# kchmck/p25rx

Measured on NVIDIA B200. Metric: Msamples/s IQ demod+decode (real-time P25 channels = baseband samples/s / 48000), higher is better.
Workload: dtype f32

## Files before the change

p25rx_b200/csrc/ddc_fm.cu:

```cuda
#include "p25cu_internal.cuh"
#include "p25_imma_tables.h"

__constant__ float c_taps_front[P25_TAPS_FRONT];
__constant__ float c_taps_decim[P25_TAPS_DECIM];
__constant__ float c_taps_chan[P25_TAPS_CHAN];
__constant__ float c_iq_lut[256];

static_assert(P25_TAPS_FRONT == 5 * P25_DECIM_FRONT, "front stage is a 10-phase x 5-tap polyphase matrix");
static_assert(P25_TAPS_DECIM == 5 * P25_DECIM_NATIVE, "decimator is a 5-phase x 5-tap polyphase matrix");

template <bool FRONT>
struct Cfg {
    static constexpr int MB = FRONT ? 64 : 256;
    static constexpr int NT = FRONT ? 320 : 256;
    static constexpr int DIN = FRONT ? 50 : 5;
    static constexpr int XN = MB * DIN;
    static constexpr int ACOLS = FRONT ? 5 * MB : 0;
    static constexpr int RING = FRONT ? 128 : 512;
    static constexpr int HT = FRONT ? 3264 : 1312;
};

template <bool FRONT>
struct Smem {
    using C = Cfg<FRONT>;
    float2 xs[C::XN];
    float2 pa[2][4][FRONT ? C::ACOLS : 1];
    float ya_re[FRONT ? C::ACOLS : 1], ya_im[FRONT ? C::ACOLS : 1];
    float2 pd[2][4][C::MB];
    float yd_re[C::RING], yd_im[C::RING];
    float c_re[C::RING], c_im[C::RING];
    float d[C::RING];
    float red[32];
    float lut[256];
};

template <int FMT>
struct Elem { using T = float2; };
template <>
struct Elem<P25CU_FMT_U8_IQ> { using T = uchar2; };

template <int FMT>
__device__ __forceinline__ float2 cvt(const float* lut, typename Elem<FMT>::T v) {
    if constexpr (FMT == P25CU_FMT_CF32_IQ) return v;
    else return make_float2(lut[v.x], lut[v.y]);
}

template <int FMT>
__device__ __forceinline__ typename Elem<FMT>::T load_logical_raw(const DdcParams& p, const void* tail, const void* chunk, long long l) {
    using T = typename Elem<FMT>::T;
    if (l < (long long)p.ht) return ((const T*)tail)[l];
    const long long i = l - p.ht;
    if (i >= (long long)p.n) return T{};
    return __ldcs((const T*)chunk + i);
}

template <bool FRONT, int FMT>
__device__ __forceinline__ void stage_block(Smem<FRONT>& sm, const DdcParams& p, const void* tail, const void* chunk,
                                            long long l0) {
    using C = Cfg<FRONT>;
    const long long ht = (long long)p.ht;
    const int tid = threadIdx.x;
    const long long t_end = l0 + C::XN < ht ? l0 + C::XN : ht;
    if (l0 < t_end) {
        if constexpr (FMT == P25CU_FMT_CF32_IQ) {
            for (long long l = (l0 & ~1LL) + 2 * tid; l < t_end; l += 2 * C::NT) {
                const float4 v = *(const float4*)((const float2*)tail + l);
                const long long i = l - l0;
                if (i >= 0) sm.xs[i] = make_float2(v.x, v.y);
                if (i + 1 < C::XN && l + 1 < t_end) sm.xs[i + 1] = make_float2(v.z, v.w);
            }
        } else {
            const long long zero_below = ht - (long long)p.a0;
            for (long long l = l0 + tid; l < t_end; l += C::NT) {
                const uchar2 b = ((const uchar2*)tail)[l];
                sm.xs[l - l0] = l < zero_below ? make_float2(0.f, 0.f) : make_float2(sm.lut[b.x], sm.lut[b.y]);
            }
        }
    }
    const long long c_beg = (l0 > ht ? l0 : ht) - ht, c_end = l0 + C::XN - ht;
    if (c_end <= c_beg) return;
    const long long base = ht - l0;
    const long long n = (long long)p.n;
    if (p.aligned16) {
        if (FMT == P25CU_FMT_CF32_IQ) {
            for (long long g = (c_beg & ~1LL) + 2 * tid; g < c_end; g += 2 * C::NT) {
                const float4 v = g < n ? __ldcs((const float4*)((const float2*)chunk + g)) : make_float4(0.f, 0.f, 0.f, 0.f);
                if (g >= c_beg) sm.xs[g + base] = make_float2(v.x, v.y);
                if (g + 1 < c_end) sm.xs[g + 1 + base] = make_float2(v.z, v.w);
            }
        } else {
            for (long long g = (c_beg & ~7LL) + 8 * tid; g < c_end; g += 8 * C::NT) {
                const uint4 v = g < n ? __ldcs((const uint4*)((const uchar2*)chunk + g)) : make_uint4(0x7F7F7F7Fu, 0x7F7F7F7Fu, 0x7F7F7F7Fu, 0x7F7F7F7Fu);
                const unsigned w[4] = {v.x, v.y, v.z, v.w};
#pragma unroll
                for (int e = 0; e < 8; e++) {
                    const long long jj = g + e;
                    if (jj >= c_beg && jj < c_end) {
                        const unsigned b = w[e >> 1] >> (16 * (e & 1));
                        sm.xs[jj + base] = jj < n ? make_float2(sm.lut[b & 0xFF], sm.lut[(b >> 8) & 0xFF]) : make_float2(0.f, 0.f);
                    }
                }
            }
        }
    } else {
        for (long long jj = c_beg + tid; jj < c_end; jj += C::NT) {
            float2 v = make_float2(0.f, 0.f);
            if (jj < n) v = cvt<FMT>(sm.lut, __ldcs((const typename Elem<FMT>::T*)chunk + jj));
            sm.xs[jj + base] = v;
        }
    }
}

template <int D>
__device__ __forceinline__ void column_partials(const float2 (&x)[D], const float* __restrict__ h, float2 (&P)[5]) {
#pragma unroll
    for (int q = 0; q < 5; q++) {
        float re = 0.f, im = 0.f;
#pragma unroll
        for (int pp = 0; pp < D; pp++) {
            const float t = h[D * q + pp];
            re = fmaf(t, x[D - 1 - pp].x, re);
            im = fmaf(t, x[D - 1 - pp].y, im);
        }
        P[q] = make_float2(re, im);
    }
}

template <bool FRONT, int FMT>
__global__ void __launch_bounds__(Cfg<FRONT>::NT) p25_ddc_fm_kernel(const DdcParams p) {
    using C = Cfg<FRONT>;
    extern __shared__ __align__(16) unsigned char smem_raw[];
    Smem<FRONT>& sm = *reinterpret_cast<Smem<FRONT>*>(smem_raw);
    const int tid = threadIdx.x;
    const unsigned s = blockIdx.x / p.n_seg, g = blockIdx.x % p.n_seg;

    {
        float* z = reinterpret_cast<float*>(&sm.pa[0][0][0]);
        const int nz = (int)((sizeof(Smem<FRONT>) - sizeof(sm.xs) - sizeof(sm.lut)) / sizeof(float));
        for (int i = tid; i < nz; i += C::NT) z[i] = 0.f;
        for (int i = tid; i < 256; i += C::NT) sm.lut[i] = c_iq_lut[i];
    }

    using ET = typename Elem<FMT>::T;
    const void* tail = (const ET*)p.tail_in + (size_t)s * p.ht;
    const void* chunk = (FMT == P25CU_FMT_CF32_IQ) ? (const void*)((const float2*)p.iq + (size_t)s * p.n)
                                                    : (const void*)((const uchar2*)p.iq + (size_t)s * p.n);
    float* out = p.bb + (size_t)s * p.row_stride + P25CU_BB_HIST;

    const long long M0 = (long long)p.m0;
    const long long mb = M0 + (long long)g * p.seg_out;
    long long me = mb + p.seg_out;
    if (me > M0 + (long long)p.n_out) me = M0 + p.n_out;
    const long long a0 = (long long)p.a0;
    float pw = 0.f;
    int pb = 0;
    __syncthreads();

    for (long long mi = mb - C::MB; mi < me; mi += C::MB, pb ^= 1) {
        stage_block<FRONT, FMT>(sm, p, tail, chunk, (long long)C::DIN * mi - a0 + (long long)p.ht);
        __syncthreads();

        if constexpr (FRONT) {
            float2 P[5];
            {
                float2 x[10];
                const float4* src = reinterpret_cast<const float4*>(&sm.xs[10 * tid]);
#pragma unroll
                for (int i = 0; i < 5; i++) {
                    const float4 v = src[i];
                    x[2 * i] = make_float2(v.x, v.y);
                    x[2 * i + 1] = make_float2(v.z, v.w);
                }
                column_partials<10>(x, c_taps_front, P);
            }
#pragma unroll
            for (int q = 1; q < 5; q++) sm.pa[pb][q - 1][tid] = P[q];
            __syncthreads();
            float re = P[0].x, im = P[0].y;
#pragma unroll
            for (int q = 1; q < 5; q++) {
                const int c = tid - q;
                const float2 v = c >= 0 ? sm.pa[pb][q - 1][c] : sm.pa[pb ^ 1][q - 1][C::ACOLS + c];
                re += v.x;
                im += v.y;
            }
            sm.ya_re[tid] = re;
            sm.ya_im[tid] = im;
            __syncthreads();
        }

        float2 Q[5];
        if (tid < C::MB) {
            float2 x[5];
            if constexpr (FRONT) {
#pragma unroll
                for (int i = 0; i < 5; i++) x[i] = make_float2(sm.ya_re[5 * tid + i], sm.ya_im[5 * tid + i]);
            } else {
#pragma unroll
                for (int i = 0; i < 5; i++) x[i] = sm.xs[5 * tid + i];
            }
            column_partials<5>(x, c_taps_decim, Q);
#pragma unroll
            for (int q = 1; q < 5; q++) sm.pd[pb][q - 1][tid] = Q[q];
        }
        __syncthreads();
        if (tid < C::MB) {
            float re = Q[0].x, im = Q[0].y;
#pragma unroll
            for (int q = 1; q < 5; q++) {
                const int c = tid - q;
                const float2 v = c >= 0 ? sm.pd[pb][q - 1][c] : sm.pd[pb ^ 1][q - 1][C::MB + c];
                re += v.x;
                im += v.y;
            }
            const unsigned r = (unsigned)(mi + tid) & (C::RING - 1);
            sm.yd_re[r] = re;
            sm.yd_im[r] = im;
        }
        __syncthreads();

        for (int w = tid; w < 2 * C::MB; w += C::NT) {
            const int o = w < C::MB ? w : w - C::MB;
            const float* src = w < C::MB ? sm.yd_re : sm.yd_im;
            const unsigned r = (unsigned)(mi + o);
            float acc = 0.f;
#pragma unroll
            for (int k = 0; k < P25_TAPS_CHAN; k++) acc = fmaf(c_taps_chan[k], src[(r - k) & (C::RING - 1)], acc);
            (w < C::MB ? sm.c_re : sm.c_im)[r & (C::RING - 1)] = acc;
        }
        __syncthreads();

        if (tid < C::MB) {
            const long long m = mi + tid;
            const unsigned r = (unsigned)m;
            const float cr = sm.c_re[r & (C::RING - 1)], ci = sm.c_im[r & (C::RING - 1)];
            const float pr = sm.c_re[(r - 1) & (C::RING - 1)], pi = sm.c_im[(r - 1) & (C::RING - 1)];
            const float re = cr * pr + ci * pi;
            const float im = ci * pr - cr * pi;
            sm.d[r & (C::RING - 1)] = atan2f(im, re) * P25_FM_GAIN;
            if (m >= mb && m < me) pw += cr * cr + ci * ci;
        }
        __syncthreads();

        if (tid < C::MB) {
            const long long m = mi + tid;
            if (m >= mb && m < me) {
                const unsigned r = (unsigned)m;
                float acc = 0.f;
#pragma unroll
                for (int i = P25_BOXCAR - 1; i >= 0; i--) acc += sm.d[(r - i) & (C::RING - 1)];
                out[m - M0] = acc / (float)P25_BOXCAR;
            }
        }
    }

    if (p.power_sum) {
#pragma unroll
        for (int o = 16; o > 0; o >>= 1) pw += __shfl_xor_sync(0xFFFFFFFFu, pw, o);
        __syncthreads();
        if ((tid & 31) == 0) sm.red[tid >> 5] = pw;
        __syncthreads();
        if (tid == 0) {
            float t = 0.f;
            for (int i = 0; i < C::NT / 32; i++) t += sm.red[i];
            atomicAdd(p.power_sum + s, t);
        }
    }

    if (g == p.n_seg - 1) {
        ET* tout = (ET*)p.tail_out + (size_t)s * p.ht;
        for (int i = tid; i < (int)p.ht; i += C::NT) tout[i] = load_logical_raw<FMT>(p, tail, chunk, (long long)p.n + i);
    }
}

namespace fast {

constexpr int MB = 64;
constexpr int NT = 320;
constexpr int XN = MB * 50;
constexpr int ACOLS = 5 * MB;
constexpr int HC = P25_TAPS_CHAN - 1;
constexpr int HB = P25_BOXCAR - 1;

template <int FMT>
struct F {
    static constexpr bool U8 = FMT == P25CU_FMT_U8_IQ;
    static constexpr int ES = U8 ? 2 : 8;
    static constexpr int AL = U8 ? 8 : 2;
    static constexpr int XLEN = U8 ? XN + AL : XN;
    static constexpr int XBYTES = (XLEN * ES + 127) / 128 * 128;
#ifndef DDC50_MAXREG
#define DDC50_MAXREG 56
#endif
#ifndef DDC50_U8_MAXREG
#define DDC50_U8_MAXREG 48
#endif
    static constexpr int MAXREG = U8 ? DDC50_U8_MAXREG : DDC50_MAXREG;
};

template <int FMT>
struct __align__(128) Smem {
    unsigned char xs[2][F<FMT>::XBYTES];
    float2 pa[4][ACOLS + 4];
    float2 ya[ACOLS];
    float2 pd[4][MB + 4];
    float2 yd[HC + MB];
    float2 c[1 + MB];
    float d[HB + MB];
    float red[16];
    unsigned long long full[2];
};

__device__ __forceinline__ unsigned smem_u32(const void* p) { return (unsigned)__cvta_generic_to_shared(p); }
__device__ __forceinline__ void mbar_init(unsigned long long* bar, unsigned count) {
    asm volatile("mbarrier.init.shared::cta.b64 [%0], %1;" ::"r"(smem_u32(bar)), "r"(count));
}
__device__ __forceinline__ void mbar_expect_tx(unsigned long long* bar, unsigned bytes) {
    asm volatile("mbarrier.arrive.expect_tx.shared::cta.b64 _, [%0], %1;" ::"r"(smem_u32(bar)), "r"(bytes) : "memory");
}
__device__ __forceinline__ void mbar_wait(unsigned long long* bar, unsigned parity) {
    unsigned ok;
    do {
        asm volatile(
            "{\n\t.reg .pred p;\n\tmbarrier.try_wait.parity.shared::cta.b64 p, [%1], %2;\n\tselp.u32 %0, 1, 0, p;\n\t}"
            : "=r"(ok)
            : "r"(smem_u32(bar)), "r"(parity)
            : "memory");
    } while (!ok);
}
__device__ __forceinline__ void tma_load_1d(void* dst, const void* src, unsigned bytes, unsigned long long* bar) {
    asm volatile("cp.async.bulk.shared::cluster.global.mbarrier::complete_tx::bytes [%0], [%1], %2, [%3];" ::"r"(smem_u32(dst)),
                 "l"(src), "r"(bytes), "r"(smem_u32(bar))
                 : "memory");
}
__device__ __forceinline__ float2 cfma(float h, float2 x, float2 acc) {
    unsigned long long r;
    const float2 hh = make_float2(h, h);
    asm("fma.rn.f32x2 %0, %1, %2, %3;"
        : "=l"(r)
        : "l"(*reinterpret_cast<const unsigned long long*>(&hh)), "l"(*reinterpret_cast<const unsigned long long*>(&x)),
          "l"(*reinterpret_cast<const unsigned long long*>(&acc)));
    return *reinterpret_cast<float2*>(&r);
}
__device__ __forceinline__ float2 add2(float2 a, float2 b) {
    unsigned long long r;
    asm("add.rn.f32x2 %0, %1, %2;"
        : "=l"(r)
        : "l"(*reinterpret_cast<const unsigned long long*>(&a)), "l"(*reinterpret_cast<const unsigned long long*>(&b)));
    return *reinterpret_cast<float2*>(&r);
}

template <int NS, bool ODD>
__device__ __forceinline__ void load_u8n(const unsigned* __restrict__ wp, float2 (&x)[NS]) {
    constexpr int NWORD = (NS + (ODD ? 1 : 0) + 1) / 2;
    unsigned w[NWORD];
#pragma unroll
    for (int i = 0; i < NWORD; i++) w[i] = wp[i];
    const float2 off = make_float2(-8388736.f, -8388736.f);
#pragma unroll
    for (int i = 0; i < NS; i++) {
        const int hw = i + (ODD ? 1 : 0);
        const unsigned word = w[hw >> 1];
        const unsigned fi = __byte_perm(word, 0x4B000000u, (hw & 1) ? 0x7442u : 0x7440u);
        const unsigned fq = __byte_perm(word, 0x4B000000u, (hw & 1) ? 0x7443u : 0x7441u);
        x[i] = add2(make_float2(__uint_as_float(fi), __uint_as_float(fq)), off);
    }
}

template <int D>
__device__ __forceinline__ void partials(const float2 (&x)[D], const float* __restrict__ h, float2 (&P)[5]) {
#pragma unroll
    for (int q = 0; q < 5; q++) {
        float2 a = make_float2(0.f, 0.f);
#pragma unroll
        for (int pp = 0; pp < D; pp++) a = cfma(h[D * q + pp], x[D - 1 - pp], a);
        P[q] = a;
    }
}

template <int FMT>
__device__ __forceinline__ void issue_block(Smem<FMT>& sm, int stage, const DdcParams& p, const unsigned char* tail,
                                            const unsigned char* chunk, long long l0) {
    constexpr int ES = F<FMT>::ES;
    const long long ht = p.ht, lend = ht + (long long)p.n;
    const long long la = l0 & ~(long long)(F<FMT>::AL - 1);
    long long l1 = la + F<FMT>::XLEN;
    if (l1 > lend) l1 = lend;
    const long long t1 = l1 < ht ? l1 : ht;
    const unsigned nt = la < t1 ? (unsigned)(t1 - la) : 0u;
    const long long cb = la > ht ? la : ht;
    const unsigned nc = cb < l1 ? (unsigned)(l1 - cb) : 0u;
    mbar_expect_tx(&sm.full[stage], (nt + nc) * ES);
    if (nt) tma_load_1d(&sm.xs[stage][0], tail + la * ES, nt * ES, &sm.full[stage]);
    if (nc) tma_load_1d(&sm.xs[stage][(cb - la) * ES], chunk + (cb - ht) * ES, nc * ES, &sm.full[stage]);
}

#ifndef DDC50_DYN_CH
#define DDC50_DYN_CH 16
#endif
#ifndef DDC50_STATIC_NUM
#define DDC50_STATIC_NUM 7
#define DDC50_STATIC_DEN 8
#endif
constexpr unsigned DYN_CH = DDC50_DYN_CH;

template <int FMT>
__global__ void __maxnreg__(F<FMT>::MAXREG) p25_ddc_fm_stream_kernel(const DdcParams p, const unsigned blocks_per_stream,
                                                                    const unsigned n_static, const unsigned n_tickets,
                                                                    const unsigned ticket_base, const float dc, const float pw_scale) {
    constexpr int ES = F<FMT>::ES;
    extern __shared__ __align__(128) unsigned char smem_raw[];
    Smem<FMT>& sm = *reinterpret_cast<Smem<FMT>*>(smem_raw);
    __shared__ unsigned s_ticket;
    const int tid = threadIdx.x;

    if (tid == 0) {
        mbar_init(&sm.full[0], 1);
        mbar_init(&sm.full[1], 1);
        asm volatile("fence.mbarrier_init.release.cluster;" ::: "memory");
    }
    const unsigned long long total = (unsigned long long)p.n_streams * blocks_per_stream;
    const unsigned long long dyn_begin = (unsigned long long)n_static * gridDim.x;
    unsigned long long b = (unsigned long long)n_static * blockIdx.x;
    unsigned long long b_end = b + n_static;
    const long long M0 = (long long)p.m0, a0 = (long long)p.a0;
    unsigned use = 0;
    __syncthreads();

  for (;;) {
    if (b >= b_end) {
        if (tid == 0) s_ticket = atomicAdd(p.work_counter, 1u) - ticket_base;
        __syncthreads();
        const unsigned c = s_ticket;
        __syncthreads();
        if (c >= n_tickets) break;
        b = dyn_begin + (unsigned long long)c * DYN_CH;
        b_end = b + DYN_CH < total ? b + DYN_CH : total;
    }
    while (b < b_end) {
        const unsigned s = (unsigned)(b / blocks_per_stream);
        const unsigned it0 = (unsigned)(b % blocks_per_stream);
        unsigned it1 = blocks_per_stream;
        if (b_end - b < (unsigned long long)(it1 - it0)) it1 = it0 + (unsigned)(b_end - b);
        b += it1 - it0;
        const unsigned char* tail = (const unsigned char*)p.tail_in + (size_t)s * p.ht * ES;
        const unsigned char* chunk = (const unsigned char*)p.iq + (size_t)s * p.n * ES;
        const long long mb = M0 + (long long)it0 * MB;
        long long me = M0 + (long long)it1 * MB;
        if (me > M0 + (long long)p.n_out) me = M0 + p.n_out;
        float* out = p.bb + (size_t)s * p.row_stride + P25CU_BB_HIST - M0;
        const long long lbase = -a0 + (long long)p.ht;

        for (int i = tid; i < 4 * 4; i += NT) {
            sm.pa[i >> 2][i & 3] = make_float2(0.f, 0.f);
            sm.pd[i >> 2][i & 3] = make_float2(0.f, 0.f);
        }
        for (int i = tid; i < HC; i += NT) sm.yd[i] = make_float2(0.f, 0.f);
        if (tid == 0) sm.c[0] = make_float2(0.f, 0.f);
        if (tid < HB) sm.d[tid] = 0.f;
        float pw = 0.f;
        const long long m_first = mb - MB;
        const int nblk = (int)((me - m_first + MB - 1) / MB);
        if (tid == 0) {
            issue_block<FMT>(sm, use & 1, p, tail, chunk, 50 * m_first + lbase);
            if (nblk > 1) issue_block<FMT>(sm, (use + 1) & 1, p, tail, chunk, 50 * (m_first + MB) + lbase);
        }
        __syncthreads();

        for (int blk = 0; blk < nblk; blk++, use++) {
            const long long mi = m_first + (long long)blk * MB;
            const int stage = use & 1;
            mbar_wait(&sm.full[stage], (use >> 1) & 1);

            float2 P[5];
            {
                float2 x[10];
                if constexpr (F<FMT>::U8) {
                    const int s0 = (int)((50 * mi + lbase) & (F<FMT>::AL - 1)) + 10 * tid;
                    const unsigned* wp = reinterpret_cast<const unsigned*>(sm.xs[stage]) + (s0 >> 1);
                    if (s0 & 1) load_u8n<10, true>(wp, x);
                    else load_u8n<10, false>(wp, x);
                } else {
                    const float4* src = reinterpret_cast<const float4*>(sm.xs[stage]) + 5 * tid;
#pragma unroll
                    for (int i = 0; i < 5; i++) {
                        const float4 v = src[i];
                        x[2 * i] = make_float2(v.x, v.y);
                        x[2 * i + 1] = make_float2(v.z, v.w);
                    }
                }
                partials<10>(x, c_taps_front, P);
            }
#pragma unroll
            for (int q = 1; q < 5; q++) sm.pa[q - 1][tid + 4] = P[q];
            __syncthreads();
            if (tid == 0 && blk + 2 < nblk) issue_block<FMT>(sm, stage, p, tail, chunk, 50 * (mi + 2 * MB) + lbase);
            {
                float2 a = P[0];
#pragma unroll
                for (int q = 1; q < 5; q++) {
                    const float2 v = sm.pa[q - 1][tid + 4 - q];
                    a.x += v.x;
                    a.y += v.y;
                }
                sm.ya[tid] = a;
            }
            __syncthreads();
            if (tid >= ACOLS - 4) {
#pragma unroll
                for (int q = 1; q < 5; q++) sm.pa[q - 1][tid - (ACOLS - 4)] = P[q];
            }
            float2 Q[5];
            if (tid < MB) {
                float2 x[5];
#pragma unroll
                for (int i = 0; i < 5; i++) x[i] = sm.ya[5 * tid + i];
                partials<5>(x, c_taps_decim, Q);
#pragma unroll
                for (int q = 1; q < 5; q++) sm.pd[q - 1][tid + 4] = Q[q];
            }
            __syncthreads();
            if (tid < MB) {
                float2 a = Q[0];
#pragma unroll
                for (int q = 1; q < 5; q++) {
                    const float2 v = sm.pd[q - 1][tid + 4 - q];
                    a.x += v.x;
                    a.y += v.y;
                }
                sm.yd[HC + tid] = a;
            }
            __syncthreads();
            if (tid >= MB - 4 && tid < MB) {
#pragma unroll
                for (int q = 1; q < 5; q++) sm.pd[q - 1][tid - (MB - 4)] = Q[q];
            }
            if (tid < MB) {
                float2 e = make_float2(dc, dc), o = make_float2(0.f, 0.f);
                const float2* src = &sm.yd[HC + tid];
#pragma unroll
                for (int k = 0; k + 1 < P25_TAPS_CHAN; k += 2) {
                    e = cfma(c_taps_chan[k], src[-k], e);
                    o = cfma(c_taps_chan[k + 1], src[-k - 1], o);
                }
                e = cfma(c_taps_chan[P25_TAPS_CHAN - 1], src[-(P25_TAPS_CHAN - 1)], e);
                sm.c[1 + tid] = make_float2(e.x + o.x, e.y + o.y);
            }
            __syncthreads();
            if (tid < MB) {
                const float2 cur = sm.c[1 + tid], prv = sm.c[tid];
                const float re = cur.x * prv.x + cur.y * prv.y;
                const float im = cur.y * prv.x - cur.x * prv.y;
                sm.d[HB + tid] = atan2f(im, re) * P25_FM_GAIN;
                const long long m = mi + tid;
                if (m >= mb && m < me) pw += cur.x * cur.x + cur.y * cur.y;
            } else if (tid >= 128 && tid < 128 + HC) {
                sm.yd[tid - 128] = sm.yd[MB + tid - 128];
            }
            __syncthreads();
            float bsum = 0.f;
            if (tid < MB) {
#pragma unroll
                for (int i = 0; i < P25_BOXCAR; i++) bsum += sm.d[tid + i];
                const long long m = mi + tid;
                if (m >= mb && m < me) out[m] = bsum / (float)P25_BOXCAR;
            } else if (tid == 128) {
                sm.c[0] = sm.c[MB];
            }
            __syncthreads();
            if (tid < HB) sm.d[tid] = sm.d[MB + tid];
        }

        if (p.power_sum) {
#pragma unroll
            for (int o = 16; o > 0; o >>= 1) pw += __shfl_xor_sync(0xFFFFFFFFu, pw, o);
            if ((tid & 31) == 0) sm.red[tid >> 5] = pw;
            __syncthreads();
            if (tid == 0) {
                float t = 0.f;
                for (int i = 0; i < NT / 32; i++) t += sm.red[i];
                atomicAdd(p.power_sum + s, t * pw_scale);
            }
        }
        if (it1 == blocks_per_stream) {
            using ET = typename Elem<FMT>::T;
            ET* tout = (ET*)p.tail_out + (size_t)s * p.ht;
            for (int i = tid; i < (int)p.ht; i += NT)
                tout[i] = load_logical_raw<FMT>(p, tail, chunk, (long long)p.n + i);
        }
        __syncthreads();
    }
  }
}

__device__ __forceinline__ float2 mul2(float2 a, float2 b) {
    unsigned long long r;
    asm("mul.rn.f32x2 %0, %1, %2;"
        : "=l"(r)
        : "l"(*reinterpret_cast<const unsigned long long*>(&a)), "l"(*reinterpret_cast<const unsigned long long*>(&b)));
    return *reinterpret_cast<float2*>(&r);
}
__device__ __forceinline__ float2 fma2s(float2 a, float2 b, float c) {
    unsigned long long r;
    const float2 cc = make_float2(c, c);
    asm("fma.rn.f32x2 %0, %1, %2, %3;"
        : "=l"(r)
        : "l"(*reinterpret_cast<const unsigned long long*>(&a)), "l"(*reinterpret_cast<const unsigned long long*>(&b)),
          "l"(*reinterpret_cast<const unsigned long long*>(&cc)));
    return *reinterpret_cast<float2*>(&r);
}
__device__ __forceinline__ float2 disc_atan2_pair(float2 y, float2 x) {
    const float ax0 = fabsf(x.x), ay0 = fabsf(y.x), ax1 = fabsf(x.y), ay1 = fabsf(y.y);
    const float mx0 = fmaxf(ax0, ay0), mn0 = fminf(ax0, ay0), mx1 = fmaxf(ax1, ay1), mn1 = fminf(ax1, ay1);
    float rc0, rc1;
    asm("rcp.approx.ftz.f32 %0, %1;" : "=f"(rc0) : "f"(fmaxf(mx0, 1e-30f)));
    asm("rcp.approx.ftz.f32 %0, %1;" : "=f"(rc1) : "f"(fmaxf(mx1, 1e-30f)));
    const float2 t = mul2(make_float2(mn0, mn1), make_float2(rc0, rc1)), u = mul2(t, t);
    float2 q = make_float2(-0.004295386839658022f, -0.004295386839658022f);
    q = fma2s(q, u, 0.022737378254532814f);
    q = fma2s(q, u, -0.057179518043994904f);
    q = fma2s(q, u, 0.09735459089279175f);
    q = fma2s(q, u, -0.13945257663726807f);
    q = fma2s(q, u, 0.1995391547679901f);
    q = fma2s(q, u, -0.3333050608634949f);
    q = fma2s(q, u, 0.9999995231628418f);
    const float2 r = mul2(q, t);
    float r0 = r.x, r1 = r.y;
    r0 = ay0 > ax0 ? 1.57079632679489662f - r0 : r0;
    r1 = ay1 > ax1 ? 1.57079632679489662f - r1 : r1;
    r0 = x.x < 0.f ? 3.14159265358979324f - r0 : r0;
    r1 = x.y < 0.f ? 3.14159265358979324f - r1 : r1;
    return make_float2(copysignf(r0, y.x), copysignf(r1, y.y));
}

}


namespace w5 {

using fast::cfma;
using fast::mbar_init;
using fast::mbar_expect_tx;
using fast::mbar_wait;
using fast::tma_load_1d;
using fast::add2;
using fast::disc_atan2_pair;

constexpr int R = 4;
constexpr int NOUT = 31 * R;
constexpr int XNEW = 5 * NOUT;
constexpr int XN = 32 * 5 * R;
constexpr int WARPS = 4;
constexpr int AL = 2, ES = 8;
constexpr int XLEN = (XN + 2 * AL - 2) / AL * AL;
constexpr int XBYTES = (XLEN * ES + 127) / 128 * 128;
constexpr int MINB = 4;
constexpr int HROWS = (P25_TAPS_CHAN - 1) / R;
constexpr int DROWS = 3;
static_assert((P25_TAPS_CHAN - 1) % R == 0 && DROWS * R >= P25_BOXCAR - 1, "history rows");

struct __align__(128) WarpSm {
    unsigned char xs[2][XBYTES];
    float4 ydA[HROWS + 32], ydB[HROWS + 32];
    float4 d4[DROWS + 32];
    unsigned long long full[2];
};

__device__ __forceinline__ void issue_slice(WarpSm& sm, int stage, int ht, int lend, const unsigned char* tail,
                                            const unsigned char* chunk, int l0) {
    const int la = l0 & ~(AL - 1);
    const int lb = min(la + XLEN, lend);
    if (la >= ht) {
        const unsigned bytes = (unsigned)(lb - la) * ES;
        mbar_expect_tx(&sm.full[stage], bytes);
        tma_load_1d(&sm.xs[stage][0], chunk + (size_t)(la - ht) * ES, bytes, &sm.full[stage]);
        return;
    }
    const int t1 = min(lb, ht);
    const unsigned nt = (unsigned)(t1 - la), nc = (unsigned)(lb - t1);
    mbar_expect_tx(&sm.full[stage], (nt + nc) * ES);
    tma_load_1d(&sm.xs[stage][0], tail + (size_t)la * ES, nt * ES, &sm.full[stage]);
    if (nc) tma_load_1d(&sm.xs[stage][nt * ES], chunk, nc * ES, &sm.full[stage]);
}

__global__ void __launch_bounds__(32 * WARPS, MINB) p25_ddc5_warp_kernel(const DdcParams p, const unsigned its_per_stream,
                                                                         const float dc, const float pw_scale) {
    extern __shared__ __align__(128) unsigned char smem_raw[];
    const int lane = threadIdx.x & 31, warp = threadIdx.x >> 5;
    WarpSm& sm = reinterpret_cast<WarpSm*>(smem_raw)[warp];
    if (lane == 0) {
        mbar_init(&sm.full[0], 1);
        mbar_init(&sm.full[1], 1);
        asm volatile("fence.mbarrier_init.release.cluster;" ::: "memory");
    }
    for (int i = lane; i < HROWS + 32; i += 32) sm.ydA[i] = sm.ydB[i] = make_float4(0.f, 0.f, 0.f, 0.f);
    for (int i = lane; i < DROWS + 32; i += 32) sm.d4[i] = make_float4(0.f, 0.f, 0.f, 0.f);
    __syncwarp();

    const unsigned gw = blockIdx.x * WARPS + warp, GW = gridDim.x * WARPS;
    const unsigned long long total = (unsigned long long)p.n_streams * its_per_stream;
    const unsigned long long b0 = total * gw / GW, b1 = total * (gw + 1ull) / GW;
    if (b0 >= b1) return;
    const int ips = (int)its_per_stream, ht = (int)p.ht, lend = (int)p.ht + (int)p.n, n_out = (int)p.n_out;
    const size_t row_bytes = (size_t)p.n * ES, tail_bytes = (size_t)p.ht * ES;
    const int l_base = (int)(5 * (long long)p.m0 - (long long)p.a0) - 20 + ht;
    const bool want_pw = p.power_sum != nullptr;
    unsigned s = (unsigned)(b0 / its_per_stream);
    int it_first = (int)(b0 % its_per_stream);
    unsigned left = (unsigned)(b1 - b0);
    const unsigned char* chunk = (const unsigned char*)p.iq + s * row_bytes;
    const unsigned char* tail = (const unsigned char*)p.tail_in + s * tail_bytes;
    if (lane == 0) {
        issue_slice(sm, 0, ht, lend, tail, chunk, l_base + XNEW * (it_first - 1));
        issue_slice(sm, 1, ht, lend, tail, chunk, l_base + XNEW * it_first);
    }
    float2 c_carry = make_float2(0.f, 0.f);
    unsigned use = 0;

    while (left) {
      const int n_st = min(ips - it_first, (int)left);
      const int npiece = n_st + 1;
      left -= (unsigned)n_st;
      float* const out_lane = p.bb + (size_t)s * p.row_stride + P25CU_BB_HIST + R * lane;
      float pw = 0.f;
      for (int j = 0; j < npiece; j++, use++) {
        const int it = it_first - 1 + j;
        const int stage = use & 1;
        const int skew = (l_base + XNEW * it) & (AL - 1);
        const int nv = j ? min(n_out - NOUT * it, NOUT) : 0;
        mbar_wait(&sm.full[stage], (use >> 1) & 1);

        float2 own[R];
        {
            float2 x[5 * R];
            const int s0 = skew + 5 * R * lane;
            const float4* xp = reinterpret_cast<const float4*>(reinterpret_cast<const float2*>(sm.xs[stage]) + (s0 & ~1));
            if (s0 & 1) {
#pragma unroll
                for (int i = 0; i <= 5 * R / 2; i++) {
                    const float4 v = xp[i];
                    if (i > 0) x[2 * i - 1] = make_float2(v.x, v.y);
                    if (i < 5 * R / 2) x[2 * i] = make_float2(v.z, v.w);
                }
            } else {
#pragma unroll
                for (int i = 0; i < 5 * R / 2; i++) {
                    const float4 v = xp[i];
                    x[2 * i] = make_float2(v.x, v.y);
                    x[2 * i + 1] = make_float2(v.z, v.w);
                }
            }
            float2 lft[R];
#pragma unroll
            for (int r = 0; r < R; r++) {
                own[r] = make_float2(0.f, 0.f);
                lft[r] = make_float2(0.f, 0.f);
#pragma unroll
                for (int k = P25_TAPS_DECIM - 1; k >= 0; k--) {
                    if ((P25_TAPS_DECIM_ZERO_MASK >> k) & 1) continue;
                    const int idx = 5 * r + (P25_TAPS_DECIM - 1) - k;
                    if (idx < 5 * R) own[r] = cfma(c_taps_decim[k], x[idx], own[r]);
                    else lft[r] = cfma(c_taps_decim[k], x[idx - 5 * R], lft[r]);
                }
            }
#pragma unroll
            for (int r = 0; r < R; r++) {
                if (5 * r + (P25_TAPS_DECIM - 1) >= 5 * R) {
                    own[r].x += __shfl_down_sync(0xFFFFFFFFu, lft[r].x, 1);
                    own[r].y += __shfl_down_sync(0xFFFFFFFFu, lft[r].y, 1);
                }
            }
        }
        sm.ydA[HROWS + lane] = make_float4(own[0].x, own[0].y, own[1].x, own[1].y);
        sm.ydB[HROWS + lane] = make_float4(own[2].x, own[2].y, own[3].x, own[3].y);
        __syncwarp();
        if (lane == 0) {
            if (j + 2 < npiece) issue_slice(sm, stage, ht, lend, tail, chunk, l_base + XNEW * (it + 2));
            else if (left) issue_slice(sm, stage, ht, lend, tail + tail_bytes, chunk + row_bytes, l_base + XNEW * (j + 1 - npiece));
        }

        float2 acc[R];
#pragma unroll
        for (int r = 0; r < R; r++) acc[r] = make_float2(dc, dc);
#pragma unroll
        for (int t = 0; t <= HROWS; t++) {
            const float4 va = sm.ydA[lane + t], vb = sm.ydB[lane + t];
            const float2 xs4[4] = {make_float2(va.x, va.y), make_float2(va.z, va.w), make_float2(vb.x, vb.y), make_float2(vb.z, vb.w)};
#pragma unroll
            for (int q = 0; q < 4; q++) {
#pragma unroll
                for (int r = 0; r < R; r++) {
                    const int k = (P25_TAPS_CHAN - 1) + r - (4 * t + q);
                    if (k >= 0 && k < P25_TAPS_CHAN) acc[r] = cfma(c_taps_chan[k], xs4[q], acc[r]);
                }
            }
        }
        float2 prev;
        prev.x = __shfl_up_sync(0xFFFFFFFFu, acc[R - 1].x, 1);
        prev.y = __shfl_up_sync(0xFFFFFFFFu, acc[R - 1].y, 1);
        if (lane == 0) prev = c_carry;
        c_carry.x = __shfl_sync(0xFFFFFFFFu, acc[R - 1].x, 30);
        c_carry.y = __shfl_sync(0xFFFFFFFFu, acc[R - 1].y, 30);
        float dd[R];
        static_assert(R % 2 == 0, "the discriminator runs on output pairs");
#pragma unroll
        for (int r = 0; r < R; r += 2) {
            const float2 c0 = acc[r], c1 = acc[r + 1];
            const float2 re = make_float2(c0.x * prev.x + c0.y * prev.y, c1.x * c0.x + c1.y * c0.y);
            const float2 im = make_float2(c0.y * prev.x - c0.x * prev.y, c1.y * c0.x - c1.x * c0.y);
            const float2 th = disc_atan2_pair(im, re);
            dd[r] = th.x * P25_FM_GAIN;
            dd[r + 1] = th.y * P25_FM_GAIN;
            if (want_pw && R * lane + r < nv) pw += c0.x * c0.x + c0.y * c0.y;
            if (want_pw && R * lane + r + 1 < nv) pw += c1.x * c1.x + c1.y * c1.y;
            prev = c1;
        }
        sm.d4[DROWS + lane] = make_float4(dd[0], dd[1], dd[2], dd[3]);
        __syncwarp();

        {
            const float a = sm.d4[lane].w;
            const float4 b = sm.d4[lane + 1], c4 = sm.d4[lane + 2];
            float s0 = a + b.x;
            s0 += b.y; s0 += b.z; s0 += b.w; s0 += c4.x; s0 += c4.y; s0 += c4.z; s0 += c4.w; s0 += dd[0];
            const float s1 = (s0 - a) + dd[1], s2 = (s1 - b.x) + dd[2], s3 = (s2 - b.y) + dd[3];
            const float kk = 1.0f / P25_BOXCAR;
            const int o0 = R * lane;
            if (o0 < nv) {
                float* out = out_lane + NOUT * it;
                if (o0 + 3 < nv) *reinterpret_cast<float4*>(out) = make_float4(s0 * kk, s1 * kk, s2 * kk, s3 * kk);
                else {
                    out[0] = s0 * kk;
                    if (o0 + 1 < nv) out[1] = s1 * kk;
                    if (o0 + 2 < nv) out[2] = s2 * kk;
                }
            }
        }
        float4 ra = make_float4(0.f, 0.f, 0.f, 0.f), rb = ra, rd = ra;
        if (lane < HROWS) {
            ra = sm.ydA[31 + lane];
            rb = sm.ydB[31 + lane];
        }
        if (lane < DROWS) rd = sm.d4[31 + lane];
        __syncwarp();
        if (lane < HROWS) {
            sm.ydA[lane] = ra;
            sm.ydB[lane] = rb;
        }
        if (lane < DROWS) sm.d4[lane] = rd;

      }
      if (want_pw) {
#pragma unroll
          for (int o = 16; o > 0; o >>= 1) pw += __shfl_xor_sync(0xFFFFFFFFu, pw, o);
          if (lane == 0) atomicAdd(p.power_sum + s, pw * pw_scale);
      }
      if (it_first + n_st == ips) {
          const uint4* src = reinterpret_cast<const uint4*>(chunk + ((size_t)p.n - p.ht) * ES);
          uint4* dst = reinterpret_cast<uint4*>((unsigned char*)p.tail_out + s * tail_bytes);
          for (int i = lane; i < (int)(tail_bytes / 16); i += 32) dst[i] = src[i];
      }
      s++;
      it_first = 0;
      chunk += row_bytes;
      tail += tail_bytes;
    }
}

}


namespace w5i {

using fast::mbar_init;
using fast::mbar_expect_tx;
using fast::mbar_wait;
using fast::tma_load_1d;
using fast::cfma;
using fast::add2;
using fast::disc_atan2_pair;

constexpr int R = 8;
constexpr int NOUT = 32 * R;
constexpr int XNEW = 5 * NOUT;
constexpr int XREAD = 5 * (NOUT - 1) + P25_TAPS_DECIM;
constexpr int WARPS = 4;
constexpr int AL = 8, ES = 2;
constexpr int XLEN = (XREAD + 2 * AL - 2) / AL * AL;
constexpr int XBYTES = (XLEN * ES + 127) / 128 * 128;
constexpr int MINB = 4;
constexpr int HROWS = (P25_TAPS_CHAN - 1) / R;
constexpr int YROWS = HROWS + 32;
constexpr int DROWS = 2;
constexpr int NB = 18;
constexpr int SCALE_LOG2 = 25;
static_assert(XLEN * ES >= 80 * 31 + 8 + 128 && XNEW % (2 * AL) == 0, "A rows inside the slice; constant skew");
static_assert((P25_TAPS_CHAN - 1) % R == 0 && DROWS * R >= P25_BOXCAR - 1 && (YROWS * 4) % 8 == 4, "history rows, store banks");

struct __align__(128) WarpSm {
    unsigned char xs[2][XBYTES];
    float4 yd[4][YROWS];
    float4 dA[DROWS + 32], dB[DROWS + 32];
    unsigned long long full[2];
};

__device__ uint2 g_btab[4][NB][32];
__device__ int4 g_init[3];

__device__ __forceinline__ void imma(int (&d)[4], const unsigned (&a)[4], const uint2 b) {
    asm("mma.sync.aligned.m16n8k32.row.col.s32.u8.s8.s32 {%0,%1,%2,%3}, {%4,%5,%6,%7}, {%8,%9}, {%0,%1,%2,%3};"
        : "+r"(d[0]), "+r"(d[1]), "+r"(d[2]), "+r"(d[3])
        : "r"(a[0]), "r"(a[1]), "r"(a[2]), "r"(a[3]), "r"(b.x), "r"(b.y));
}
__device__ __forceinline__ void imma0(int (&d)[4], const unsigned (&a)[4], const uint2 b, const int (&c)[4]) {
    asm("mma.sync.aligned.m16n8k32.row.col.s32.u8.s8.s32 {%0,%1,%2,%3}, {%4,%5,%6,%7}, {%8,%9}, {%10,%11,%12,%13};"
        : "=r"(d[0]), "=r"(d[1]), "=r"(d[2]), "=r"(d[3])
        : "r"(a[0]), "r"(a[1]), "r"(a[2]), "r"(a[3]), "r"(b.x), "r"(b.y), "r"(c[0]), "r"(c[1]), "r"(c[2]), "r"(c[3]));
}
__device__ __forceinline__ unsigned lds32(unsigned addr) {
    unsigned v;
    asm volatile("ld.shared.u32 %0, [%1];" : "=r"(v) : "r"(addr));
    return v;
}

__device__ __forceinline__ void issue_slice(WarpSm& sm, int stage, int ht, int lend, const unsigned char* tail,
                                            const unsigned char* chunk, int l0) {
    const int la = l0 & ~(AL - 1);
    const int lb = min(la + XLEN, lend);
    if (la >= ht) {
        const unsigned bytes = (unsigned)(lb - la) * ES;
        mbar_expect_tx(&sm.full[stage], bytes);
        tma_load_1d(&sm.xs[stage][0], chunk + (size_t)(la - ht) * ES, bytes, &sm.full[stage]);
        return;
    }
    const int t1 = min(lb, ht);
    const unsigned nt = (unsigned)(t1 - la), nc = (unsigned)(lb - t1);
// ... 624 lines not shown
```

Baseline: 757,500.

## Use warp shuffles and named barriers in fast DDC stream kernel

Rewrites the polyphase partial-sum combination to use warp shuffles with small per-warp boundary buffers (double-buffered by stage) instead of full shared arrays. After the front stage, the warps that are not needed exit the block iteration early and the remaining two warps synchronise with a named 64-thread barrier rather than block-wide __syncthreads. It also replaces atan2f with a polynomial approximation, skips known-zero decimator taps, and vectorises the tail copy with 16-byte streaming loads. The cost is more complex boundary handling and the risk of small numerical differences from the approximate atan.

```diff
diff --git a/p25rx_b200/csrc/ddc_fm.cu b/p25rx_b200/csrc/ddc_fm.cu
--- a/p25rx_b200/csrc/ddc_fm.cu
+++ b/p25rx_b200/csrc/ddc_fm.cu
@@ -281,6 +281,7 @@
 constexpr int ACOLS = 5 * MB;
 constexpr int HC = P25_TAPS_CHAN - 1;
 constexpr int HB = P25_BOXCAR - 1;
+constexpr int NW = NT / 32;
 
 template <int FMT>
 struct F {
@@ -301,9 +302,9 @@
 template <int FMT>
 struct __align__(128) Smem {
     unsigned char xs[2][F<FMT>::XBYTES];
-    float2 pa[4][ACOLS + 4];
     float2 ya[ACOLS];
-    float2 pd[4][MB + 4];
+    float2 pb[2][NW][4][4];
+    float2 qb[2][2][4][4];
     float2 yd[HC + MB];
     float2 c[1 + MB];
     float d[HB + MB];
@@ -348,249 +349,6 @@
         : "=l"(r)
         : "l"(*reinterpret_cast<const unsigned long long*>(&a)), "l"(*reinterpret_cast<const unsigned long long*>(&b)));
     return *reinterpret_cast<float2*>(&r);
-}
-
-template <int NS, bool ODD>
-__device__ __forceinline__ void load_u8n(const unsigned* __restrict__ wp, float2 (&x)[NS]) {
-    constexpr int NWORD = (NS + (ODD ? 1 : 0) + 1) / 2;
-    unsigned w[NWORD];
-#pragma unroll
-    for (int i = 0; i < NWORD; i++) w[i] = wp[i];
-    const float2 off = make_float2(-8388736.f, -8388736.f);
-#pragma unroll
-    for (int i = 0; i < NS; i++) {
-        const int hw = i + (ODD ? 1 : 0);
-        const unsigned word = w[hw >> 1];
-        const unsigned fi = __byte_perm(word, 0x4B000000u, (hw & 1) ? 0x7442u : 0x7440u);
-        const unsigned fq = __byte_perm(word, 0x4B000000u, (hw & 1) ? 0x7443u : 0x7441u);
-        x[i] = add2(make_float2(__uint_as_float(fi), __uint_as_float(fq)), off);
-    }
-}
-
-template <int D>
-__device__ __forceinline__ void partials(const float2 (&x)[D], const float* __restrict__ h, float2 (&P)[5]) {
-#pragma unroll
-    for (int q = 0; q < 5; q++) {
-        float2 a = make_float2(0.f, 0.f);
-#pragma unroll
-        for (int pp = 0; pp < D; pp++) a = cfma(h[D * q + pp], x[D - 1 - pp], a);
-        P[q] = a;
-    }
-}
-
-template <int FMT>
-__device__ __forceinline__ void issue_block(Smem<FMT>& sm, int stage, const DdcParams& p, const unsigned char* tail,
-                                            const unsigned char* chunk, long long l0) {
-    constexpr int ES = F<FMT>::ES;
-    const long long ht = p.ht, lend = ht + (long long)p.n;
-    const long long la = l0 & ~(long long)(F<FMT>::AL - 1);
-    long long l1 = la + F<FMT>::XLEN;
-    if (l1 > lend) l1 = lend;
-    const long long t1 = l1 < ht ? l1 : ht;
-    const unsigned nt = la < t1 ? (unsigned)(t1 - la) : 0u;
-    const long long cb = la > ht ? la : ht;
-    const unsigned nc = cb < l1 ? (unsigned)(l1 - cb) : 0u;
-    mbar_expect_tx(&sm.full[stage], (nt + nc) * ES);
-    if (nt) tma_load_1d(&sm.xs[stage][0], tail + la * ES, nt * ES, &sm.full[stage]);
-    if (nc) tma_load_1d(&sm.xs[stage][(cb - la) * ES], chunk + (cb - ht) * ES, nc * ES, &sm.full[stage]);
-}
-
-#ifndef DDC50_DYN_CH
-#define DDC50_DYN_CH 16
-#endif
-#ifndef DDC50_STATIC_NUM
-#define DDC50_STATIC_NUM 7
-#define DDC50_STATIC_DEN 8
-#endif
-constexpr unsigned DYN_CH = DDC50_DYN_CH;
-
-template <int FMT>
-__global__ void __maxnreg__(F<FMT>::MAXREG) p25_ddc_fm_stream_kernel(const DdcParams p, const unsigned blocks_per_stream,
-                                                                    const unsigned n_static, const unsigned n_tickets,
-                                                                    const unsigned ticket_base, const float dc, const float pw_scale) {
-    constexpr int ES = F<FMT>::ES;
-    extern __shared__ __align__(128) unsigned char smem_raw[];
-    Smem<FMT>& sm = *reinterpret_cast<Smem<FMT>*>(smem_raw);
-    __shared__ unsigned s_ticket;
-    const int tid = threadIdx.x;
-
-    if (tid == 0) {
-        mbar_init(&sm.full[0], 1);
-        mbar_init(&sm.full[1], 1);
-        asm volatile("fence.mbarrier_init.release.cluster;" ::: "memory");
-    }
-    const unsigned long long total = (unsigned long long)p.n_streams * blocks_per_stream;
-    const unsigned long long dyn_begin = (unsigned long long)n_static * gridDim.x;
-    unsigned long long b = (unsigned long long)n_static * blockIdx.x;
-    unsigned long long b_end = b + n_static;
-    const long long M0 = (long long)p.m0, a0 = (long long)p.a0;
-    unsigned use = 0;
-    __syncthreads();
-
-  for (;;) {
-    if (b >= b_end) {
-        if (tid == 0) s_ticket = atomicAdd(p.work_counter, 1u) - ticket_base;
-        __syncthreads();
-        const unsigned c = s_ticket;
-        __syncthreads();
-        if (c >= n_tickets) break;
-        b = dyn_begin + (unsigned long long)c * DYN_CH;
-        b_end = b + DYN_CH < total ? b + DYN_CH : total;
-    }
-    while (b < b_end) {
-        const unsigned s = (unsigned)(b / blocks_per_stream);
-        const unsigned it0 = (unsigned)(b % blocks_per_stream);
-        unsigned it1 = blocks_per_stream;
-        if (b_end - b < (unsigned long long)(it1 - it0)) it1 = it0 + (unsigned)(b_end - b);
-        b += it1 - it0;
-        const unsigned char* tail = (const unsigned char*)p.tail_in + (size_t)s * p.ht * ES;
-        const unsigned char* chunk = (const unsigned char*)p.iq + (size_t)s * p.n * ES;
-        const long long mb = M0 + (long long)it0 * MB;
-        long long me = M0 + (long long)it1 * MB;
-        if (me > M0 + (long long)p.n_out) me = M0 + p.n_out;
-        float* out = p.bb + (size_t)s * p.row_stride + P25CU_BB_HIST - M0;
-        const long long lbase = -a0 + (long long)p.ht;
-
-        for (int i = tid; i < 4 * 4; i += NT) {
-            sm.pa[i >> 2][i & 3] = make_float2(0.f, 0.f);
-            sm.pd[i >> 2][i & 3] = make_float2(0.f, 0.f);
-        }
-        for (int i = tid; i < HC; i += NT) sm.yd[i] = make_float2(0.f, 0.f);
-        if (tid == 0) sm.c[0] = make_float2(0.f, 0.f);
-        if (tid < HB) sm.d[tid] = 0.f;
-        float pw = 0.f;
-        const long long m_first = mb - MB;
-        const int nblk = (int)((me - m_first + MB - 1) / MB);
-        if (tid == 0) {
-            issue_block<FMT>(sm, use & 1, p, tail, chunk, 50 * m_first + lbase);
-            if (nblk > 1) issue_block<FMT>(sm, (use + 1) & 1, p, tail, chunk, 50 * (m_first + MB) + lbase);
-        }
-        __syncthreads();
-
-        for (int blk = 0; blk < nblk; blk++, use++) {
-            const long long mi = m_first + (long long)blk * MB;
-            const int stage = use & 1;
-            mbar_wait(&sm.full[stage], (use >> 1) & 1);
-
-            float2 P[5];
-            {
-                float2 x[10];
-                if constexpr (F<FMT>::U8) {
-                    const int s0 = (int)((50 * mi + lbase) & (F<FMT>::AL - 1)) + 10 * tid;
-                    const unsigned* wp = reinterpret_cast<const unsigned*>(sm.xs[stage]) + (s0 >> 1);
-                    if (s0 & 1) load_u8n<10, true>(wp, x);
-                    else load_u8n<10, false>(wp, x);
-                } else {
-                    const float4* src = reinterpret_cast<const float4*>(sm.xs[stage]) + 5 * tid;
-#pragma unroll
-                    for (int i = 0; i < 5; i++) {
-                        const float4 v = src[i];
-                        x[2 * i] = make_float2(v.x, v.y);
-                        x[2 * i + 1] = make_float2(v.z, v.w);
-                    }
-                }
-                partials<10>(x, c_taps_front, P);
-            }
-#pragma unroll
-            for (int q = 1; q < 5; q++) sm.pa[q - 1][tid + 4] = P[q];
-            __syncthreads();
-            if (tid == 0 && blk + 2 < nblk) issue_block<FMT>(sm, stage, p, tail, chunk, 50 * (mi + 2 * MB) + lbase);
-            {
-                float2 a = P[0];
-#pragma unroll
-                for (int q = 1; q < 5; q++) {
-                    const float2 v = sm.pa[q - 1][tid + 4 - q];
-                    a.x += v.x;
-                    a.y += v.y;
-                }
-                sm.ya[tid] = a;
-            }
-            __syncthreads();
-            if (tid >= ACOLS - 4) {
-#pragma unroll
-                for (int q = 1; q < 5; q++) sm.pa[q - 1][tid - (ACOLS - 4)] = P[q];
-            }
-            float2 Q[5];
-            if (tid < MB) {
-                float2 x[5];
-#pragma unroll
-                for (int i = 0; i < 5; i++) x[i] = sm.ya[5 * tid + i];
-                partials<5>(x, c_taps_decim, Q);
-#pragma unroll
-                for (int q = 1; q < 5; q++) sm.pd[q - 1][tid + 4] = Q[q];
-            }
-            __syncthreads();
-            if (tid < MB) {
-                float2 a = Q[0];
-#pragma unroll
-                for (int q = 1; q < 5; q++) {
-                    const float2 v = sm.pd[q - 1][tid + 4 - q];
-                    a.x += v.x;
-                    a.y += v.y;
-                }
-                sm.yd[HC + tid] = a;
-            }
-            __syncthreads();
-            if (tid >= MB - 4 && tid < MB) {
-#pragma unroll
-                for (int q = 1; q < 5; q++) sm.pd[q - 1][tid - (MB - 4)] = Q[q];
-            }
-            if (tid < MB) {
-                float2 e = make_float2(dc, dc), o = make_float2(0.f, 0.f);
-                const float2* src = &sm.yd[HC + tid];
-#pragma unroll
-                for (int k = 0; k + 1 < P25_TAPS_CHAN; k += 2) {
-                    e = cfma(c_taps_chan[k], src[-k], e);
-                    o = cfma(c_taps_chan[k + 1], src[-k - 1], o);
-                }
-                e = cfma(c_taps_chan[P25_TAPS_CHAN - 1], src[-(P25_TAPS_CHAN - 1)], e);
-                sm.c[1 + tid] = make_float2(e.x + o.x, e.y + o.y);
-            }
-            __syncthreads();
-            if (tid < MB) {
-                const float2 cur = sm.c[1 + tid], prv = sm.c[tid];
-                const float re = cur.x * prv.x + cur.y * prv.y;
-                const float im = cur.y * prv.x - cur.x * prv.y;
-                sm.d[HB + tid] = atan2f(im, re) * P25_FM_GAIN;
-                const long long m = mi + tid;
-                if (m >= mb && m < me) pw += cur.x * cur.x + cur.y * cur.y;
-            } else if (tid >= 128 && tid < 128 + HC) {
-                sm.yd[tid - 128] = sm.yd[MB + tid - 128];
-            }
-            __syncthreads();
-            float bsum = 0.f;
-            if (tid < MB) {
-#pragma unroll
-                for (int i = 0; i < P25_BOXCAR; i++) bsum += sm.d[tid + i];
-                const long long m = mi + tid;
-                if (m >= mb && m < me) out[m] = bsum / (float)P25_BOXCAR;
-            } else if (tid == 128) {
-                sm.c[0] = sm.c[MB];
-            }
-            __syncthreads();
-            if (tid < HB) sm.d[tid] = sm.d[MB + tid];
-        }
-
-        if (p.power_sum) {
-#pragma unroll
-            for (int o = 16; o > 0; o >>= 1) pw += __shfl_xor_sync(0xFFFFFFFFu, pw, o);
-            if ((tid & 31) == 0) sm.red[tid >> 5] = pw;
-            __syncthreads();
-            if (tid == 0) {
-                float t = 0.f;
-                for (int i = 0; i < NT / 32; i++) t += sm.red[i];
-                atomicAdd(p.power_sum + s, t * pw_scale);
-            }
-        }
-        if (it1 == blocks_per_stream) {
-            using ET = typename Elem<FMT>::T;
-            ET* tout = (ET*)p.tail_out + (size_t)s * p.ht;
-            for (int i = tid; i < (int)p.ht; i += NT)
-                tout[i] = load_logical_raw<FMT>(p, tail, chunk, (long long)p.n + i);
-        }
-        __syncthreads();
-    }
-  }
 }
 
 __device__ __forceinline__ float2 mul2(float2 a, float2 b) {
@@ -632,6 +390,273 @@
     r1 = x.y < 0.f ? 3.14159265358979324f - r1 : r1;
     return make_float2(copysignf(r0, y.x), copysignf(r1, y.y));
 }
+__device__ __forceinline__ void bar_sync(unsigned id, unsigned n) { asm volatile("bar.sync %0, %1;" ::"r"(id), "r"(n) : "memory"); }
+__device__ __forceinline__ float2 shfl_up2(float2 v, unsigned d) {
+    return make_float2(__shfl_up_sync(0xFFFFFFFFu, v.x, d), __shfl_up_sync(0xFFFFFFFFu, v.y, d));
+}
+
+template <int NS, bool ODD>
+__device__ __forceinline__ void load_u8n(const unsigned* __restrict__ wp, float2 (&x)[NS]) {
+    constexpr int NWORD = (NS + (ODD ? 1 : 0) + 1) / 2;
+    unsigned w[NWORD];
+#pragma unroll
+    for (int i = 0; i < NWORD; i++) w[i] = wp[i];
+    const float2 off = make_float2(-8388736.f, -8388736.f);
+#pragma unroll
+    for (int i = 0; i < NS; i++) {
+        const int hw = i + (ODD ? 1 : 0);
+        const unsigned word = w[hw >> 1];
+        const unsigned fi = __byte_perm(word, 0x4B000000u, (hw & 1) ? 0x7442u : 0x7440u);
+        const unsigned fq = __byte_perm(word, 0x4B000000u, (hw & 1) ? 0x7443u : 0x7441u);
+        x[i] = add2(make_float2(__uint_as_float(fi), __uint_as_float(fq)), off);
+    }
+}
+
+template <int D, unsigned ZERO = 0u>
+__device__ __forceinline__ void partials(const float2 (&x)[D], const float* __restrict__ h, float2 (&P)[5]) {
+#pragma unroll
+    for (int q = 0; q < 5; q++) {
+        float2 a = make_float2(0.f, 0.f);
+#pragma unroll
+        for (int pp = 0; pp < D; pp++)
+            if (!((ZERO >> (D * q + pp)) & 1u)) a = cfma(h[D * q + pp], x[D - 1 - pp], a);
+        P[q] = a;
+    }
+}
+
+template <int FMT>
+__device__ __forceinline__ void issue_block(Smem<FMT>& sm, int stage, const DdcParams& p, const unsigned char* tail,
+                                            const unsigned char* chunk, long long l0) {
+    constexpr int ES = F<FMT>::ES;
+    const long long ht = p.ht, lend = ht + (long long)p.n;
+    const long long la = l0 & ~(long long)(F<FMT>::AL - 1);
+    long long l1 = la + F<FMT>::XLEN;
+    if (l1 > lend) l1 = lend;
+    const long long t1 = l1 < ht ? l1 : ht;
+    const unsigned nt = la < t1 ? (unsigned)(t1 - la) : 0u;
+    const long long cb = la > ht ? la : ht;
+    const unsigned nc = cb < l1 ? (unsigned)(l1 - cb) : 0u;
+    mbar_expect_tx(&sm.full[stage], (nt + nc) * ES);
+    if (nt) tma_load_1d(&sm.xs[stage][0], tail + la * ES, nt * ES, &sm.full[stage]);
+    if (nc) tma_load_1d(&sm.xs[stage][(cb - la) * ES], chunk + (cb - ht) * ES, nc * ES, &sm.full[stage]);
+}
+
+#ifndef DDC50_DYN_CH
+#define DDC50_DYN_CH 16
+#endif
+#ifndef DDC50_STATIC_NUM
+#define DDC50_STATIC_NUM 7
+#define DDC50_STATIC_DEN 8
+#endif
+constexpr unsigned DYN_CH = DDC50_DYN_CH;
+
+template <int FMT>
+__global__ void __maxnreg__(F<FMT>::MAXREG) p25_ddc_fm_stream_kernel(const DdcParams p, const unsigned blocks_per_stream,
+                                                                    const unsigned n_static, const unsigned n_tickets,
+                                                                    const unsigned ticket_base, const float dc, const float pw_scale) {
+    constexpr int ES = F<FMT>::ES;
+    extern __shared__ __align__(128) unsigned char smem_raw[];
+    Smem<FMT>& sm = *reinterpret_cast<Smem<FMT>*>(smem_raw);
+    __shared__ unsigned s_ticket;
+    const int tid = threadIdx.x;
+
+    if (tid == 0) {
+        mbar_init(&sm.full[0], 1);
+        mbar_init(&sm.full[1], 1);
+        asm volatile("fence.mbarrier_init.release.cluster;" ::: "memory");
+    }
+    const unsigned long long total = (unsigned long long)p.n_streams * blocks_per_stream;
+    const unsigned long long dyn_begin = (unsigned long long)n_static * gridDim.x;
+    unsigned long long b = (unsigned long long)n_static * blockIdx.x;
+    unsigned long long b_end = b + n_static;
+    const long long M0 = (long long)p.m0, a0 = (long long)p.a0;
+    unsigned use = 0;
+    __syncthreads();
+
+  for (;;) {
+    if (b >= b_end) {
+        if (tid == 0) s_ticket = atomicAdd(p.work_counter, 1u) - ticket_base;
+        __syncthreads();
+        const unsigned c = s_ticket;
+        __syncthreads();
+        if (c >= n_tickets) break;
+        b = dyn_begin + (unsigned long long)c * DYN_CH;
+        b_end = b + DYN_CH < total ? b + DYN_CH : total;
+    }
+    while (b < b_end) {
+        const unsigned s = (unsigned)(b / blocks_per_stream);
+        const unsigned it0 = (unsigned)(b % blocks_per_stream);
+        unsigned it1 = blocks_per_stream;
+        if (b_end - b < (unsigned long long)(it1 - it0)) it1 = it0 + (unsigned)(b_end - b);
+        b += it1 - it0;
+        const unsigned char* tail = (const unsigned char*)p.tail_in + (size_t)s * p.ht * ES;
+        const unsigned char* chunk = (const unsigned char*)p.iq + (size_t)s * p.n * ES;
+        const long long mb = M0 + (long long)it0 * MB;
+        long long me = M0 + (long long)it1 * MB;
+        if (me > M0 + (long long)p.n_out) me = M0 + p.n_out;
+        float* out = p.bb + (size_t)s * p.row_stride + P25CU_BB_HIST - M0;
+        const long long lbase = -a0 + (long long)p.ht;
+
+        const int lane = tid & 31, warp = tid >> 5;
+        for (int i = tid; i < 4 * 4; i += NT) {
+            sm.pb[(use & 1) ^ 1][NW - 1][i >> 2][i & 3] = make_float2(0.f, 0.f);
+            sm.qb[(use & 1) ^ 1][1][i >> 2][i & 3] = make_float2(0.f, 0.f);
+        }
+        for (int i = tid; i < HC; i += NT) sm.yd[i] = make_float2(0.f, 0.f);
+        if (tid == 0) sm.c[0] = make_float2(0.f, 0.f);
+        if (tid < HB) sm.d[tid] = 0.f;
+        float pw = 0.f;
+        const long long m_first = mb - MB;
+        const int nblk = (int)((me - m_first + MB - 1) / MB);
+        if (tid == 0) {
+            issue_block<FMT>(sm, use & 1, p, tail, chunk, 50 * m_first + lbase);
+            if (nblk > 1) issue_block<FMT>(sm, (use + 1) & 1, p, tail, chunk, 50 * (m_first + MB) + lbase);
+        }
+        __syncthreads();
+
+        for (int blk = 0; blk < nblk; blk++, use++) {
+            const long long mi = m_first + (long long)blk * MB;
+            const int stage = use & 1;
+            mbar_wait(&sm.full[stage], (use >> 1) & 1);
+
+            float2 P[5];
+            {
+                float2 x[10];
+                if constexpr (F<FMT>::U8) {
+                    const int s0 = (int)((50 * mi + lbase) & (F<FMT>::AL - 1)) + 10 * tid;
+                    const unsigned* wp = reinterpret_cast<const unsigned*>(sm.xs[stage]) + (s0 >> 1);
+                    if (s0 & 1) load_u8n<10, true>(wp, x);
+                    else load_u8n<10, false>(wp, x);
+                } else {
+                    const float4* src = reinterpret_cast<const float4*>(sm.xs[stage]) + 5 * tid;
+#pragma unroll
+                    for (int i = 0; i < 5; i++) {
+                        const float4 v = src[i];
+                        x[2 * i] = make_float2(v.x, v.y);
+                        x[2 * i + 1] = make_float2(v.z, v.w);
+                    }
+                }
+                partials<10>(x, c_taps_front, P);
+            }
+            if (lane >= 28) {
+#pragma unroll
+                for (int q = 1; q < 5; q++) sm.pb[stage][warp][q - 1][lane - 28] = P[q];
+            }
+#pragma unroll
+            for (int q = 1; q < 5; q++) P[q] = shfl_up2(P[q], q);
+            __syncthreads();
+            if (tid == 0 && blk + 2 < nblk) issue_block<FMT>(sm, stage, p, tail, chunk, 50 * (mi + 2 * MB) + lbase);
+            {
+                if (lane < 4) {
+                    const float2(*bp)[4] = warp ? sm.pb[stage][warp - 1] : sm.pb[stage ^ 1][NW - 1];
+#pragma unroll
+                    for (int q = 1; q < 5; q++)
+                        if (lane < q) P[q] = bp[q - 1][lane + 4 - q];
+                }
+                float2 a = P[0];
+#pragma unroll
+                for (int q = 1; q < 5; q++) {
+                    a.x += P[q].x;
+                    a.y += P[q].y;
+                }
+                sm.ya[tid] = a;
+            }
+            __syncthreads();
+            if (warp >= 2) continue;
+
+            {
+                float2 Q[5];
+                {
+                    float2 x[5];
+#pragma unroll
+                    for (int i = 0; i < 5; i++) x[i] = sm.ya[5 * tid + i];
+                    partials<5, P25_TAPS_DECIM_ZERO_MASK>(x, c_taps_decim, Q);
+                }
+                if (lane >= 28) {
+#pragma unroll
+                    for (int q = 1; q < 5; q++) sm.qb[stage][warp][q - 1][lane - 28] = Q[q];
+                }
+#pragma unroll
+                for (int q = 1; q < 5; q++) Q[q] = shfl_up2(Q[q], q);
+                bar_sync(1, MB);
+                if (lane < 4) {
+                    const float2(*bq)[4] = warp ? sm.qb[stage][0] : sm.qb[stage ^ 1][1];
+#pragma unroll
+                    for (int q = 1; q < 5; q++)
+                        if (lane < q) Q[q] = bq[q - 1][lane + 4 - q];
+                }
+                float2 a = Q[0];
+#pragma unroll
+                for (int q = 1; q < 5; q++) {
+                    a.x += Q[q].x;
+                    a.y += Q[q].y;
+                }
+                sm.yd[HC + tid] = a;
+            }
+            bar_sync(1, MB);
+            {
+                float2 e = make_float2(dc, dc), o = make_float2(0.f, 0.f);
+                const float2* src = &sm.yd[HC + tid];
+#pragma unroll
+                for (int k = 0; k + 1 < P25_TAPS_CHAN; k += 2) {
+                    e = cfma(c_taps_chan[k], src[-k], e);
+                    o = cfma(c_taps_chan[k + 1], src[-k - 1], o);
+                }
+                e = cfma(c_taps_chan[P25_TAPS_CHAN - 1], src[-(P25_TAPS_CHAN - 1)], e);
+                sm.c[1 + tid] = make_float2(e.x + o.x, e.y + o.y);
+            }
+            bar_sync(1, MB);
+            {
+                const float2 cur = sm.c[1 + tid], prv = sm.c[tid];
+                const float re = cur.x * prv.x + cur.y * prv.y;
+                const float im = cur.y * prv.x - cur.x * prv.y;
+                float ph = disc_atan2_pair(make_float2(im, im), make_float2(re, re)).x;
+                if (re == 0.f && im == 0.f && signbit(re)) ph = copysignf(3.14159265358979324f, im);
+                sm.d[HB + tid] = ph * P25_FM_GAIN;
+                const long long m = mi + tid;
+                if (m >= mb && m < me) pw += cur.x * cur.x + cur.y * cur.y;
+                if (tid < HC) sm.yd[tid] = sm.yd[MB + tid];
+            }
+            bar_sync(1, MB);
+            {
+                float bsum = 0.f;
+#pragma unroll
+                for (int i = 0; i < P25_BOXCAR; i++) bsum += sm.d[tid + i];
+                const long long m = mi + tid;
+                if (m >= mb && m < me) out[m] = bsum / (float)P25_BOXCAR;
+                if (tid == 0) sm.c[0] = sm.c[MB];
+            }
+            bar_sync(1, MB);
+            if (tid < HB) sm.d[tid] = sm.d[MB + tid];
+        }
+
+        if (p.power_sum) {
+#pragma unroll
+            for (int o = 16; o > 0; o >>= 1) pw += __shfl_xor_sync(0xFFFFFFFFu, pw, o);
+            if ((tid & 31) == 0) sm.red[tid >> 5] = pw;
+            __syncthreads();
+            if (tid == 0) {
+                float t = 0.f;
+                for (int i = 0; i < NT / 32; i++) t += sm.red[i];
+                atomicAdd(p.power_sum + s, t * pw_scale);
+            }
+        }
+        if (it1 == blocks_per_stream) {
+            const size_t tail_bytes = (size_t)p.ht * ES;
+            unsigned char* tout = (unsigned char*)p.tail_out + s * tail_bytes;
+            if (p.n >= p.ht && ((p.n - p.ht) * ES) % 16 == 0) {
+                const uint4* src = reinterpret_cast<const uint4*>(chunk + (size_t)(p.n - p.ht) * ES);
+                for (int i = tid; i < (int)(tail_bytes / 16); i += NT) reinterpret_cast<uint4*>(tout)[i] = __ldcs(src + i);
+            } else {
+                using ET = typename Elem<FMT>::T;
+                for (int i = tid; i < (int)p.ht; i += NT)
+                    reinterpret_cast<ET*>(tout)[i] = load_logical_raw<FMT>(p, tail, chunk, (long long)p.n + i);
+            }
+        }
+        __syncthreads();
+    }
+  }
+}
 
 }
 
```

New measurement: 578,000 (median of 6 runs). 0.763x the previous value.
